# h2oai/datatable

Hardware: NVIDIA H100
Metric: rows/sec groupby-sum 1e9 int32 keys (higher is better)
Workload: dtype int32 keys / float64 sums

## Files before the change

### datatable_b200/csrc/dtb_api.cu

```cuda
#include <stdio.h>
#include <chrono>
#include <string.h>
#include <mutex>
#include <optional>
#include <string>
#include <vector>
#include "dtb_common.cuh"

namespace dtb {

static thread_local std::string t_error;
static thread_local dtb_call_stats t_stats = {0, 0, 0, 0, 0};

void set_error(const std::string& msg) { t_error = msg; }
void count_launch(int n) { t_stats.kernels_launched += n; }

static int64_t opt_radix_bits = 0;
static int64_t opt_verbose = 0;
static int64_t opt_profile = 0;
static int64_t opt_bucketed = 1;

struct ProfRec { const char* name; cudaEvent_t a, b; };
static thread_local std::vector<ProfRec> t_prof_open;
static thread_local std::vector<std::pair<std::string, double>> t_prof_done;
// ... 86 lines not shown
    if (slabs.size() > 1) {
      size_t total = 0;
      for (auto& sl : slabs) total += sl.cap;
      DTB_CUDA_CHECK(cudaDeviceSynchronize());
      for (auto& sl : slabs) cudaFree(sl.p);
      slabs.clear();
      char* p = nullptr;
      cudaError_t e = cudaMalloc(&p, total);
      if (e != cudaSuccess) { cudaGetLastError(); }
      else slabs.push_back({p, total});
    }
    cur = 0; off = 0;
    return DTB_OK;
  }
  void end() { if (depth > 0) depth--; }
  int take(size_t bytes, void** out) {
    bytes = (bytes + 255) & ~(size_t)255;
    while (cur < slabs.size()) {
      if (off + bytes <= slabs[cur].cap) { *out = slabs[cur].p + off; off += bytes; return DTB_OK; }
      cur++; off = 0;
    }
    size_t cap = bytes < ((size_t)64 << 20) ? ((size_t)64 << 20) : bytes;
    char* p = nullptr;
    cudaError_t e = cudaMalloc(&p, cap);
    if (e != cudaSuccess) {
      set_error("cudaMalloc(" + std::to_string(cap) + " bytes): " + cudaGetErrorString(e));
      cudaGetLastError();
      return e == cudaErrorMemoryAllocation ? DTB_ENOMEM : DTB_ECUDA;
    }
    slabs.push_back({p, cap});
// ... 258 lines not shown
  int     flags[MAX_KEYS];
  KeyPlan kp;
  int64_t nskip = 0;
  bool    groups_k = false;
  std::vector<RoundPlan> rounds;
  bool    fused_raw = false;
  int     buf_key_bytes = 4;
  int     dbits = 99;
  bool    direct_ok = false;
  bool    count_table = false;
  bool    fused_direct = false;
  int64_t ctable = 0;
  int64_t ftable = 0;
  std::vector<BucketCol> bcols;
  std::vector<int> bcol_of;
};

struct GroupBufs {
  DevIn  in[MAX_KEYS];
  const void* dptrs[MAX_KEYS];
  bool   staged = false;
  bool   fr_streamable = false;
  ColStats st[MAX_KEYS];
  DevBuf rawhist, rawna;
  DevBuf keyA, keyB, idxA, idxB, idxR0, idxR1;
  DevBuf gcount;
  DevBuf facc;
  DevBuf bxk;
  void*  sorted_keys = nullptr;
};

static int stage_inputs(const dtb_col* keys, int nkeys, int64_t n, const FusedReducers* fr, cudaStream_t s,
                        GroupBufs& b)
{
  for (int c = 0; c < nkeys; c++) {
    DTB_TRY(b.in[c].bind(keys[c].data, (size_t)n * stype_bytes(keys[c].stype), s));
    b.dptrs[c] = b.in[c].dptr;
    b.staged = b.staged || b.in[c].buf.p != nullptr;
  }
  b.fr_streamable = fr && fr->n > 0;
  for (int i = 0; b.fr_streamable && i < fr->n; i++)
    b.fr_streamable = fr->spec[i].op <= DTB_OP_NROWS &&
                       (fr->spec[i].op == DTB_OP_NROWS || is_device_ptr(fr->spec[i].value.data));
// ... 95 lines not shown
    const int np = r.pp.npasses;
    const int low = gp.count_table && np > 1 ? r.pp.shift[np - 1] : 0;
    const bool narrow = !r.want_sorted_keys && !(gp.count_table && (np > 3 || low > 16));
    r.low_bits = narrow ? low : 0;
    for (int p = 0; p < np; p++) {
      const bool lastp = p == np - 1;
      const int left = r.kp.total_bits - r.pp.shift[p] - r.pp.bits[p];
      r.kdrop[p] = narrow && p > 0 ? r.pp.shift[p] : 0;
      r.kin_bytes[p] = p == 0 ? r.key_bytes : r.kout_bytes[p - 1];
      r.kout_bytes[p] = lastp ? (r.want_sorted_keys ? r.key_bytes : 0)
                      : !narrow ? r.key_bytes : left <= 8 ? 1 : left <= 16 ? 2 : left <= 32 ? 4 : 8;
    }
    r.fold = nkeys == 1 && ri == 0 && gp.fused_raw && r.kp.k[0].cshift == 0 && r.kp.k[0].lshift == 0;
    r.keep_composite = !gp.bcols.empty() && !gp.fused_raw && nrounds == 1 && r.key_bytes == 4;
  }
}

static void print_plan(const GroupPlan& gp, int64_t n, int nkeys, const ColStats* st) {
  if (!opt_verbose) return;
  const int nrounds = (int)gp.rounds.size();
  fprintf(stderr, "[dtb200] group: n=%lld keys=%d bits=%d rounds=%d\n", (long long)n, nkeys, gp.kp.total_bits, nrounds);
  for (int c = 0; c < nkeys; c++)
    fprintf(stderr, "[dtb200]   key %d: stype=%d desc=%d bits=%d cshift=%d lshift=%d na=%llu\n", c,
            gp.kp.k[c].stype, gp.kp.k[c].desc, gp.kp.k[c].bits, gp.kp.k[c].cshift, gp.kp.k[c].lshift,
            (unsigned long long)st[c].nacount);
  for (int ri = 0; ri < nrounds; ri++) {
    const RoundPlan& r = gp.rounds[ri];
    std::string kw;
    for (int p = 0; p < r.pp.npasses; p++)
      kw += (p ? "," : "") + std::to_string(r.kin_bytes[p]) + ":" + std::to_string(r.kout_bytes[p]);
    fprintf(stderr, "[dtb200]   round %d: keys=%d bits=%d group_shift=%d passes=%d narrow_after=%d fold=%d count_table=%d"
            " key_bytes=%s low_bits=%d\n",
            ri, r.kp.nkeys, r.kp.total_bits, r.kp.group_shift, r.pp.npasses, r.narrow_after, (int)r.fold,
            (int)(gp.count_table && ri == nrounds - 1), kw.c_str(), r.low_bits);
  }
}

static int sort_rounds(const GroupPlan& gp, int64_t n, int nfused, int32_t* order, cudaStream_t s, GroupBufs& b)
{
  const int nrounds = (int)gp.rounds.size();
  DTB_TRY(b.keyA.alloc((size_t)n * gp.buf_key_bytes, s));
  DTB_TRY(b.keyB.alloc((size_t)n * gp.buf_key_bytes, s));
  DTB_TRY(b.idxA.alloc((size_t)n * 4, s));
  DTB_TRY(b.idxB.alloc((size_t)n * 4, s));
  if (nrounds > 1) { DTB_TRY(b.idxR0.alloc((size_t)n * 4, s)); }
  if (nrounds > 2) { DTB_TRY(b.idxR1.alloc((size_t)n * 4, s)); }
  if (gp.count_table) {
    DTB_TRY(b.gcount.alloc(sizeof(u32) * (size_t)gp.ctable, s));
    DTB_CUDA_CHECK(cudaMemsetAsync(b.gcount.p, 0, sizeof(u32) * (size_t)gp.ctable, s));
  }
  if (gp.fused_direct) DTB_TRY(b.facc.alloc(sizeof(u64) * (size_t)gp.ftable * 2 * (size_t)nfused, s));
  DTB_TL("scratch allocated");
  const int32_t* idx_cur = nullptr;
  for (int ri = 0; ri < nrounds; ri++) {
    const RoundPlan& r = gp.rounds[ri];
    const KeyPlan& rk = r.kp;
    const PassPlan& pp = r.pp;
    t_stats.radix_passes += pp.npasses;
    int src_kind = 1;
    if (r.keep_composite) DTB_TRY(b.bxk.alloc(sizeof(u32) * (size_t)n, s));
    if (!gp.fused_raw) {
      ProfScope ps("compose_keys", s);
      DTB_TRY(launch_compose_keys(rk, n, idx_cur, r.keep_composite ? b.bxk.p : b.keyA.p, r.key_bytes, s)); src_kind = 0;
    }

    DevBuf work; DTB_TRY(work.alloc(radix_pass_work_bytes(n), s));
// ... 16 lines not shown
      io.keys_in = kin;
      io.out_shift = last ? 0 : r.kdrop[p + 1] - r.kdrop[p];
      io.out_bytes = r.kout_bytes[p];
      if (r.fold && p == 0 && pp.shift[0] == 0) {
        io.raw_hist = b.rawhist.as<unsigned short>(); io.raw_na = b.rawna.as<unsigned short>();
      }
      if (r.low_bits) {
        if (p == 0) io.bases_out = pp.npasses == 2 ? low_base : regions;
        if (p == 1 && !last) { io.regions = regions; io.region_bits = pp.bits[0]; io.low_hist = low_base; }
        if (last) { io.low_base = low_base; io.low_bits = r.low_bits; }
      }
      io.idx_in = iin;
      io.keys_out = (last && !r.want_sorted_keys) ? nullptr : kout;
      int32_t* iout = last ? round_out : ((p & 1) ? b.idxB.as<int32_t>() : b.idxA.as<int32_t>());
      io.idx_out = iout;
      DTB_TRY(launch_radix_pass(io, rk, r.kin_bytes[p], n, pp.shift[p] - r.kdrop[p], pp.bits[p], work.as<u32>(), s,
                                (gp.count_table && last) ? b.gcount.as<u32>() : nullptr, rk.group_shift));
      if (last && r.want_sorted_keys) b.sorted_keys = kout;
      kin = kout;
      kout = (kout == b.keyA.p) ? b.keyB.p : b.keyA.p;
      iin = iout;
    }
    idx_cur = round_out;
  }
  return DTB_OK;
}

static int group_offsets(const GroupPlan& gp, int64_t n, const int32_t* order, int32_t* offsets, GroupBufs& b,
                         GroupResult& res, cudaStream_t s)
{
  if (res.ngroups < 0) return DTB_OK;
  if (!gp.groups_k) {
// ... 94 lines not shown
    const void* vals[BK_MAXCOLS]; int sts[BK_MAXCOLS]; unsigned long long* words[BK_MAXCOLS][BK_NWORDS];
    const int nc = sw.second - sw.first;
    for (int c = 0; c < nc; c++) {
      const BucketCol& bc = gp.bcols[sw.first + c];
      vals[c] = bc.data; sts[c] = bc.stype;
      for (int w = 0; w < BK_NWORDS; w++) words[c][w] = tables[(size_t)(sw.first + c) * BK_NWORDS + w];
    }
    DTB_TRY(launch_bucketed_reduce(b.bxk.as<u32>(), bshift, gp.dbits, nc, vals, sts, n, slab_starts,
                                   start, words, bscr.p, s));
  }
  return DTB_OK;
}

static int direct_reduce(const DirectGroups& dg, const DirectPlan& dp, int op, dtb_col value, const int32_t* order,
                         const int32_t* offsets, int64_t n, int64_t ng, u64* acc0, u64* acc1, bool accumulate,
                         void* out, cudaStream_t s)
{
  GroupRows rows;
  rows.v = value.data; rows.nv = n; rows.order = order; rows.offsets = offsets; rows.n = n;
  DevBuf zscr;
  if (minmax_zero_sign(op, value.stype)) { DTB_TRY(zscr.alloc(zero_fix_bytes(ng), s)); rows.zpos = zscr.as<u64>(); }
  if (accumulate && ng > 0) {
    ProfScope ps("reduce_direct", s);
    DTB_TRY(launch_direct_init(op, dp, dg.table, acc0, acc1, s));
    DTB_TRY(launch_direct_accumulate_rows(op, dg.kp, dp, value.data, value.stype, n, acc0, acc1, s));
  }
  return launch_direct_finalize(op, value.stype, acc0, acc1, dp, (const uint32_t*)dg.gkeys, ng, out, rows, s);
}

static int reduce_rowindex(int op, const void* value, int stype, int64_t nrows_value, const void* order, int order_is64,
                           const int32_t* offsets, int64_t ng, int64_t n, u64* acc, void* out, cudaStream_t s)
{
  DevBuf extra;
  const size_t xb = reduce_extra_bytes(op, stype, ng, n);
  if (xb) DTB_TRY(extra.alloc(xb, s));
  ProfScope ps("reduce", s);
  return launch_reduce_impl(op, value, stype, nrows_value, order, order_is64, offsets, ng, n, acc, acc + ng, out, s,
                            xb ? extra.p : nullptr);
}

// ... 15 lines not shown
  if (bucketed) DTB_TRY(bucketed_reduce(gp, n, b, tables, s));
  for (int i = 0; i < fr.n; i++) {
    const dtb_reduce_spec& sp = fr.spec[i];
    int out_st = 0;
    DTB_TRY(reducer_out_stype(sp.op, sp.value.stype, out_st));
    DevBuf ob; DTB_TRY(ob.alloc_owned((size_t)(ng > 0 ? ng : 1) * stype_bytes(out_st), s));
    if (sp.op == DTB_OP_NROWS) {
      DTB_TRY(launch_nrows(offsets, ng, ob.p, s));
    } else if (bucketed && gp.bcol_of[i] >= 0) {
      u64* const* w = &tables[(size_t)gp.bcol_of[i] * BK_NWORDS];
      const BucketWords bw = bucket_words(sp.op, sp.value.stype);
      DTB_TRY(direct_reduce(res.direct, dp, sp.op, sp.value, order, offsets, n, ng, w[bw.a0],
                            bw.a1 >= 0 ? w[bw.a1] : nullptr, false, ob.p, s));
    } else if (gp.fused_direct) {
      u64* acc = b.facc.as<u64>() + (size_t)gp.ftable * 2 * i;
      DTB_TRY(direct_reduce(res.direct, dp, sp.op, sp.value, order, offsets, n, ng, acc, acc + gp.ftable, true, ob.p, s));
    } else {
      DevIn dv;
      if (sp.op != DTB_OP_NROWS) DTB_TRY(dv.bind(sp.value.data, (size_t)n * stype_bytes(sp.value.stype), s));
      DTB_TRY(reduce_rowindex(sp.op, dv.dptr, sp.value.stype, n, order, 0, offsets, ng, n, gacc.as<u64>(), ob.p, s));
    }
    fr.out[i] = ob.detach();
  }
  return DTB_OK;
}

static int validate_group(const dtb_col* keys, int nkeys, const int* flags, int na_pos, int64_t n, bool handle,
                          bool wide)
{
  if (nkeys < 1 || nkeys > MAX_KEYS) { set_error("number of key columns must be in 1.." + std::to_string(MAX_KEYS)); return DTB_EINVAL; }
  if (!keys || !flags) { set_error("keys/flags must not be NULL"); return DTB_EINVAL; }
// ... 977 lines not shown
```

### datatable_b200/csrc/dtb_common.cuh

```cuda
#pragma once
#include <cuda_runtime.h>
#include <stdint.h>
#include <string.h>
#include <type_traits>
#include "dtb_internal.h"

namespace dtb {

constexpr int NUM_SMS = 132;

constexpr int PASS_THREADS = 256;
constexpr int PASS_IPT = 16;
constexpr int PASS_TILE = PASS_THREADS * PASS_IPT;
constexpr int CHUNK_TILES = 16;
constexpr int CHUNK_ROWS = PASS_TILE * CHUNK_TILES;

typedef unsigned long long u64;
typedef unsigned int u32;

template <typename T> struct NaOf;
template <> struct NaOf<int8_t>  { static __host__ __device__ int8_t  v() { return INT8_MIN;  } };
template <> struct NaOf<int16_t> { static __host__ __device__ int16_t v() { return INT16_MIN; } };
template <> struct NaOf<int32_t> { static __host__ __device__ int32_t v() { return INT32_MIN; } };
template <> struct NaOf<int64_t> { static __host__ __device__ int64_t v() { return INT64_MIN; } };
// ... 120 lines not shown
    } else {
      u64 u; const bool valid = RawKey<T>::get(r, u);
      return (KeyT)norm_apply(valid, u, k);
    }
  }
  __device__ __forceinline__ KeyT load(int64_t i) const { return norm(load_raw(i)); }
};

__device__ __forceinline__ u64 ld_relaxed_u64(const u64* p) {
  u64 v; asm volatile("ld.relaxed.gpu.global.u64 %0, [%1];" : "=l"(v) : "l"(p) : "memory"); return v;
}
__device__ __forceinline__ void st_relaxed_u64(u64* p, u64 v) {
  asm volatile("st.relaxed.gpu.global.u64 [%0], %1;" :: "l"(p), "l"(v) : "memory");
}

__device__ __forceinline__ unsigned lanemask_lt() {
  unsigned m; asm("mov.u32 %0, %%lanemask_lt;" : "=r"(m)); return m;
}

static inline int stype_bytes(int st) {
  switch (st) {
    case DTB_STYPE_BOOL: case DTB_STYPE_INT8: return 1;
    case DTB_STYPE_INT16: return 2;
    case DTB_STYPE_INT32: case DTB_STYPE_FLOAT32: case DTB_STYPE_DATE32: return 4;
    case DTB_STYPE_INT64: case DTB_STYPE_FLOAT64: case DTB_STYPE_TIME64: return 8;
    default: return 0;
  }
}

static inline int grid_for(int64_t blocks, int per_sm) {
// ... 27 lines not shown
```

### datatable_b200/csrc/dtb_internal.h

```cpp
#pragma once
#include <cuda_runtime.h>
#include <stdint.h>
#include <string>
#include "../../include/dtb200.h"

namespace dtb {

constexpr int MAX_KEYS = 8;
constexpr int MAX_PASSES = 16;

void set_error(const std::string& msg);
void count_launch(int n = 1);
struct ProfScope {
  ProfScope(const char* name, cudaStream_t s);
  ~ProfScope();
  bool on; cudaStream_t s; const char* name; cudaEvent_t a, b;
};

#define DTB_CUDA_CHECK(expr)                                                     \
  do {                                                                           \
    cudaError_t _e = (expr);                                                     \
    if (_e != cudaSuccess) {                                                     \
      ::dtb::set_error(std::string(#expr) + ": " + cudaGetErrorString(_e));      \
      return DTB_ECUDA;                                                          \
// ... 52 lines not shown
  int         src_kind;
  const void* keys_in;
  const int32_t* idx_in;
  void*       keys_out;
  int32_t*    idx_out;
  const unsigned short* raw_hist = nullptr;
  const unsigned short* raw_na = nullptr;
  int         out_shift = 0;
  int         out_bytes = 0;
  uint32_t*       bases_out = nullptr;
  const uint32_t* regions = nullptr;
  int             region_bits = 0;
  uint32_t*       low_hist = nullptr;
  const uint32_t* low_base = nullptr;
  int             low_bits = 0;
};

size_t radix_pass_work_bytes(int64_t n);
int launch_radix_pass(const PassIO& io, const KeyPlan& kp, int key_bytes, int64_t n,
                      int shift, int bits, uint32_t* work, cudaStream_t s,
                      uint32_t* group_count = nullptr, int group_shift = 0);

int launch_offsets_from_counts(const uint32_t* count, int64_t table, int64_t n, int32_t* offsets,
                               uint32_t* gkeys, unsigned long long* d_ngroups, unsigned long long* scratch,
                               cudaStream_t s);

int launch_dense_scatter(const void* keys, int key_bytes, const void* vals, int64_t n, int64_t kmin, int64_t size,
                         void* table, uint32_t* present, cudaStream_t s);
int launch_dense_emit(const uint32_t* gidx, const void* table, int64_t ng, int64_t kmin, int key_bytes,
                      void* out_keys, void* out_vals, cudaStream_t s);
// ... 18 lines not shown
size_t zero_fix_bytes(int64_t ngroups);
bool minmax_zero_sign(int op, int stype);

int launch_first_valid_pos(const void* v, int stype, int64_t nv, const void* order, int order_is64, const int32_t* offsets,
                           int64_t ngroups, int64_t n, int zero_only, const unsigned long long* gate,
                           unsigned long long* pos, cudaStream_t s);

int launch_reduce_impl(int op, const void* value, int stype, int64_t nrows_value,
                       const void* order, int order_is64, const int32_t* offsets, int64_t ngroups,
                       int64_t n, unsigned long long* acc0, unsigned long long* acc1,
                       void* out, cudaStream_t s, void* extra = nullptr);
size_t reduce_extra_bytes(int op, int stype, int64_t ng, int64_t n);
int reduce_out_stype_host(int op, int stype);
int launch_offsets_check(const int32_t* offsets, int64_t ng, int* d_bad, cudaStream_t s);

enum { DIRECT_PLAIN = 0,
       DIRECT_SMALL = 1,
       DIRECT_HOT = 2 };
struct DirectPlan {
  int kind;
  const void* map;
  int64_t nslots;
};
size_t direct_map_bytes(int64_t table);
int plan_direct(int64_t table, const uint32_t* gkeys, const int32_t* offsets, int64_t ngroups, int64_t n,
                int64_t gmax, void* map_scratch, cudaStream_t s, DirectPlan& dp);
int launch_direct_init(int op, const DirectPlan& dp, int64_t table, unsigned long long* acc0, unsigned long long* acc1, cudaStream_t s);
int launch_direct_accumulate_rows(int op, const KeyPlan& kp, const DirectPlan& dp, const void* value, int stype, int64_t n,
                                  unsigned long long* acc0, unsigned long long* acc1, cudaStream_t s);
int launch_direct_finalize(int op, int stype, const unsigned long long* acc0, const unsigned long long* acc1,
                           const DirectPlan& dp, const uint32_t* gkeys, int64_t ngroups, void* out, const GroupRows& rows,
                           cudaStream_t s);
int launch_inverse_order(const int32_t* order, int64_t n, int32_t* inv, cudaStream_t s);
int launch_first_zero_rows(const void* value_rows, int stype, int64_t row0, int64_t nrows, const int32_t* inv,
                           const int32_t* offsets, int64_t ngroups, unsigned long long* first_zero, cudaStream_t s);
int launch_nrows(const int32_t* offsets, int64_t ngroups, void* out, cudaStream_t s);
int launch_group_keys(const void* sorted_keys, int key_bytes, const int32_t* offsets, int group_shift,
                      int64_t ngroups, uint32_t* gkeys, cudaStream_t s);

enum { BK_SUMI = 0, BK_SUMF = 1, BK_CNT = 2, BK_MIN = 3, BK_MAX = 4, BK_CNTNA = 5, BK_NWORDS = 6 };
constexpr int BK_MAX_DBITS = 20, BK_MIN_DBITS = 12;
size_t bucket_starts_bytes(int64_t n);
int launch_bucket_starts(const uint32_t* xkeys, int gshift, int64_t n, int nb, uint32_t* slab_starts, uint32_t* bstart, cudaStream_t s);
constexpr int BK_MAXCOLS = 4;
// ... 56 lines not shown
```

### datatable_b200/csrc/dtb_radix.cu

```cuda
#include "dtb_common.cuh"

namespace dtb {

template <typename T>
__device__ __forceinline__ void compose_col4(const KeyNorm& k, const int64_t (&row)[4], const bool (&in)[4], u64 (&x)[4]) {
  typedef typename RawKey<T>::load_t L;
  L raw[4];
#pragma unroll
  for (int r = 0; r < 4; r++) raw[r] = in[r] ? ((const L*)k.data)[row[r]] : (L)0;
#pragma unroll
  for (int r = 0; r < 4; r++) {
    u64 u; const bool valid = RawKey<T>::get(raw[r], u);
    x[r] |= norm_apply(valid, u, k) << k.lshift;
  }
}

template <typename KeyT>
__global__ void __launch_bounds__(256)
compose_keys_kernel(KeyPlan kp, int64_t n, const int32_t* __restrict__ idx, KeyT* __restrict__ out, int out_shift)
{
  const int64_t stride = (int64_t)gridDim.x * blockDim.x * 4;
  for (int64_t i0 = (int64_t)blockIdx.x * blockDim.x * 4 + threadIdx.x; i0 < n; i0 += stride) {
    int64_t row[4]; bool in[4]; u64 x[4];
#pragma unroll
// ... 25 lines not shown
  if (key_bytes == 4 && kp.total_bits - out_shift > 32) {
    set_error("internal: a " + std::to_string(kp.total_bits - out_shift) + "-bit key does not fit 32 bits");
    return DTB_EINVAL;
  }
  if (n == 0) return DTB_OK;
  const int grid = grid_for((n + 1023) / 1024, 16);
  if (key_bytes == 4) compose_keys_kernel<u32><<<grid, 256, 0, s>>>(kp, n, idx, (u32*)keys_out, out_shift);
  else                compose_keys_kernel<u64><<<grid, 256, 0, s>>>(kp, n, idx, (u64*)keys_out, out_shift);
  count_launch();
  DTB_CUDA_CHECK(cudaGetLastError());
  return DTB_OK;
}


int64_t radix_num_chunks(int64_t n) { return (n + CHUNK_ROWS - 1) / CHUNK_ROWS; }

__device__ __forceinline__ u32 slot_owner(const u32* b, u32 lo, u32 hi, u32 s) {
  while (lo < hi) { const u32 mid = (lo + hi + 1) >> 1; if (b[mid] <= s) lo = mid; else hi = mid - 1; }
  return lo;
}

template <typename KeyT, typename Src, int NBINS>
__global__ void __launch_bounds__(PASS_THREADS)
count_kernel(const __grid_constant__ Src src, int64_t n, int shift, u32 mask, u32* __restrict__ counts,
             unsigned short* __restrict__ tile_pre, const u32* __restrict__ regions, int region_bits,
             u32* __restrict__ low_hist)
{
  constexpr int BPT = NBINS / PASS_THREADS;
  __shared__ u32 h[NBINS];
  __shared__ u32 rg[256];
  const int64_t cbase = (int64_t)blockIdx.x * CHUNK_ROWS;
  const int64_t cend = (cbase + CHUNK_ROWS < n) ? cbase + CHUNK_ROWS : n;
  const u32 rmax = (1u << region_bits) - 1;
  if (regions) { if (threadIdx.x <= rmax) rg[threadIdx.x] = regions[threadIdx.x]; }
  u32 total[BPT];
// ... 160 lines not shown
  KeyT*          keys_out;
  int32_t*       idx_out;
  int64_t        n;
  int            shift;
  u32            mask;
  const u32*     chunk_offs;
  const u32*     digit_base;
  const unsigned short* tile_pre;
  u32*           group_count;
  int            group_shift;
  int            out_shift;
  int            out_bytes;
  const u32*     low_base;
  int            low_bits;
  const uint2*   tile_low;
};

__device__ __forceinline__ void mbar_init(uint64_t* bar, u32 count) {
  const u32 a = (u32)__cvta_generic_to_shared(bar);
  asm volatile("mbarrier.init.shared::cta.b64 [%0], %1;" :: "r"(a), "r"(count) : "memory");
  asm volatile("fence.mbarrier_init.release.cluster;" ::: "memory");
}
__device__ __forceinline__ void tma_load_1d(void* smem_dst, const void* gsrc, u32 bytes, uint64_t* bar) {
  const u32 d = (u32)__cvta_generic_to_shared(smem_dst), b = (u32)__cvta_generic_to_shared(bar);
  asm volatile("mbarrier.arrive.expect_tx.shared::cta.b64 _, [%0], %1;" :: "r"(b), "r"(bytes) : "memory");
  asm volatile("cp.async.bulk.shared::cluster.global.mbarrier::complete_tx::bytes [%0], [%1], %2, [%3];"
               :: "r"(d), "l"(gsrc), "r"(bytes), "r"(b) : "memory");
}
__device__ __forceinline__ void mbar_wait(uint64_t* bar, u32 parity) {
  const u32 b = (u32)__cvta_generic_to_shared(bar);
// ... 160 lines not shown
      } else {
        skey[lp] = key[i];
        sidx[lp] = r;
      }
    }
  }
  __syncthreads();
}

template <typename KeyT>
__device__ __forceinline__ KeyT staged_key(const KeyT* skey, int q) {
  if constexpr (sizeof(KeyT) == 4) return (KeyT)reinterpret_cast<const uint2*>(skey)[q].x;
  else return skey[q];
}

template <typename KeyT, typename Src, int NBINS, int MINB, int NB>
__global__ void __launch_bounds__(PASS_THREADS, MINB)
scatter_kernel(const __grid_constant__ PassArgs<KeyT, Src> a)
{
  constexpr int THREADS = PASS_THREADS, TILE = PassCfg<KeyT, NBINS>::TILE, TILES = PassCfg<KeyT, NBINS>::TILES;
  constexpr int WARPS = THREADS / 32;
  constexpr int BPT = NBINS / THREADS;
  extern __shared__ __align__(16) unsigned char smem_raw[];
  __shared__ u32 s_wsum[WARPS];
  __shared__ __align__(8) uint64_t s_bar;
  u32* bin_dst    = reinterpret_cast<u32*>(smem_raw + sizeof(unsigned short) * WARPS * NBINS);
  KeyT* skey      = reinterpret_cast<KeyT*>(bin_dst + NBINS + 4);
  int32_t* sidx   = reinterpret_cast<int32_t*>(skey + TILE);

  const int tid = threadIdx.x;
  const int64_t base = (int64_t)blockIdx.x * TILE;
  const int tile_n = (int)((a.n - base) < (int64_t)TILE ? (a.n - base) : (int64_t)TILE);
  const int64_t tile = (int64_t)blockIdx.x * TILES;
  const int64_t chunk = tile / CHUNK_TILES;

  u32 bin_run[BPT];
#pragma unroll
  for (int j = 0; j < BPT; j++) {
    const int b = tid * BPT + j;
    bin_run[j] = a.digit_base[b] + a.chunk_offs[(size_t)chunk * NBINS + b] + (u32)a.tile_pre[(size_t)tile * NBINS + b];
  }
  uint2 tl = make_uint2(0, 0);
  if constexpr (Src::packed && sizeof(typename Src::raw_t) == 1) {
    if (a.low_base) {
      const int64_t last = tile + (tile_n - 1) / PASS_TILE;
      tl = make_uint2(a.tile_low[tile].x, a.tile_low[last].y);
    }
  }

  if (tile_n == TILE) scatter_tile<KeyT, Src, NBINS, true,  NB>(a, smem_raw, s_wsum, &s_bar, base, tile_n, bin_run, tl);
  else                scatter_tile<KeyT, Src, NBINS, false, NB>(a, smem_raw, s_wsum, &s_bar, base, tile_n, bin_run, tl);

  const int lane = tid & 31;
#pragma unroll 4
  for (int p0 = 0; p0 < tile_n; p0 += THREADS) {
    const int p = p0 + tid;
    const bool valid = p < tile_n;
    KeyT k = 0; int32_t rid = 0;
    if (valid) {
      if constexpr (sizeof(KeyT) == 4) {
        const uint2 kv = reinterpret_cast<const uint2*>(skey)[p];
        k = (KeyT)kv.x; rid = (int32_t)kv.y;
      } else {
        k = skey[p]; rid = sidx[p];
      }
    }
// ... 9 lines not shown
      }
    }
    if (valid) {
      const u32 d = (u32)(k >> a.shift) & a.mask;
      const u32 dst = bin_dst[d] + (u32)p;
      if (a.keys_out) {
        const KeyT ko = k >> a.out_shift;
        switch (a.out_bytes) {
          case 1:  reinterpret_cast<unsigned char*>(a.keys_out)[dst] = (unsigned char)ko; break;
          case 2:  reinterpret_cast<unsigned short*>(a.keys_out)[dst] = (unsigned short)ko; break;
          case 4:  reinterpret_cast<u32*>(a.keys_out)[dst] = (u32)ko; break;
          default: a.keys_out[dst] = ko; break;
        }
      }
      a.idx_out[dst] = rid;
    }
  }
}

template <typename KeyT, typename Src, int NBINS>
static int run_scatter(Src src, const PassIO& io, int64_t n, int shift, u32 mask, int64_t ntiles,
                       const u32* counts, const u32* base, const unsigned short* tile_counts,
                       u32* group_count, int group_shift, const uint2* tile_low, cudaStream_t s)
{
  constexpr int MINB = PassCfg<KeyT, NBINS>::MINB;
  PassArgs<KeyT, Src> a;
  a.src = src; a.idx_in = io.idx_in; a.keys_out = (KeyT*)io.keys_out; a.idx_out = io.idx_out;
  a.n = n; a.shift = shift + io.low_bits; a.mask = mask; a.chunk_offs = counts; a.digit_base = base;
  a.tile_pre = tile_counts; a.group_count = group_count; a.group_shift = group_shift;
  a.out_shift = io.out_shift; a.out_bytes = io.out_bytes ? io.out_bytes : (int)sizeof(KeyT);
  a.low_base = io.low_base; a.low_bits = io.low_bits; a.tile_low = tile_low;
  constexpr size_t smem = PassCfg<KeyT, NBINS>::SMEM;
  constexpr int TILE = PassCfg<KeyT, NBINS>::TILE;
  const int bits = __builtin_popcount(mask);
  void (*kern)(const PassArgs<KeyT, Src>) =
      bits <= 6 ? scatter_kernel<KeyT, Src, NBINS, MINB, 6>
    : bits == 7 ? scatter_kernel<KeyT, Src, NBINS, MINB, 7> : scatter_kernel<KeyT, Src, NBINS, MINB, 8>;
  DTB_CUDA_CHECK(cudaFuncSetAttribute(kern, cudaFuncAttributeMaxDynamicSharedMemorySize, (int)smem));
  ProfScope ps("radix_scatter", s);
  kern<<<(unsigned)((n + TILE - 1) / TILE), PASS_THREADS, smem, s>>>(a);
  count_launch();
  DTB_CUDA_CHECK(cudaGetLastError());
  return DTB_OK;
}

template <typename KeyT, typename Src, int NBINS>
static int run_pass_nb(Src src, const PassIO& io, int64_t n, int shift, int bits, u32* work, cudaStream_t s,
                       u32* group_count, int group_shift)
{
  const int64_t nchunks = radix_num_chunks(n);
  const int64_t ntiles = (n + PASS_TILE - 1) / PASS_TILE;
  u32* counts = work;
// ... 59 lines not shown
  const size_t nbins = 256;
  return sizeof(u32) * ((size_t)radix_num_chunks(n) * nbins + 2 * nbins)
       + sizeof(unsigned short) * (ntiles + CHUNK_TILES) * nbins + sizeof(uint2) * ntiles;
}

int launch_radix_pass(const PassIO& io, const KeyPlan& kp, int key_bytes, int64_t n,
                      int shift, int bits, uint32_t* work, cudaStream_t s,
                      uint32_t* group_count, int group_shift)
{
  if (bits < 1 || bits > 8) { set_error("internal: digit width must be 1..8 bits"); return DTB_EINVAL; }
  if ((io.low_base && (io.src_kind != 0 || key_bytes != 1 || io.low_bits < 1 || io.low_bits > 16)) ||
      (io.regions && (io.raw_hist || !io.low_hist || io.region_bits < 1 || io.region_bits + bits > 16)) ||
      io.out_bytes > (key_bytes == 8 ? 8 : 4)) {
    set_error("internal: bad key widths for a radix pass"); return DTB_EINVAL;
  }
  if (io.src_kind == 0) {
    switch (key_bytes) {
      case 1: { PackedSrc<unsigned char, u32> src{(const unsigned char*)io.keys_in};
        return run_pass<u32>(src, io, n, shift, bits, work, s, group_count, group_shift); }
      case 2: { PackedSrc<unsigned short, u32> src{(const unsigned short*)io.keys_in};
        return run_pass<u32>(src, io, n, shift, bits, work, s, group_count, group_shift); }
      case 4: { PackedSrc<u32> src{(const u32*)io.keys_in};
        return run_pass<u32>(src, io, n, shift, bits, work, s, group_count, group_shift); }
      default: { PackedSrc<u64> src{(const u64*)io.keys_in};
        return run_pass<u64>(src, io, n, shift, bits, work, s, group_count, group_shift); }
    }
  }
  return key_bytes == 4 ? run_pass_raw<u32>(io, kp, n, shift, bits, work, s, group_count, group_shift)
                        : run_pass_raw<u64>(io, kp, n, shift, bits, work, s, group_count, group_shift);
}
// ... 31 lines not shown
```

### datatable_b200/csrc/dtb_reduce.cu

```cuda
#include <type_traits>
#include "dtb_common.cuh"

namespace dtb {

enum { CAT_SUMI = 0, CAT_SUMF = 1, CAT_MEAN = 2, CAT_MINMAX = 3, CAT_COUNT = 4, CAT_PRODI = 5, CAT_PRODF = 6 };

constexpr int RT = 256;
constexpr int RIPT = 8;
constexpr int RTILE = RT * RIPT;

template <int CAT> struct Partial;
template <> struct Partial<CAT_SUMI> { u64 s; };
template <> struct Partial<CAT_SUMF> { double s; };
template <> struct Partial<CAT_MEAN> { double s; u32 c; };
template <> struct Partial<CAT_MINMAX> { u64 key; };
template <> struct Partial<CAT_COUNT> { u32 c; };
template <> struct Partial<CAT_PRODI> { u64 p; };
template <> struct Partial<CAT_PRODF> { double m; int64_t e; u32 f; };

constexpr u64 PRODF_FRAC = (1ull << 52) - 1;
__device__ __forceinline__ double prodf_sig(u64 w) {
  return __longlong_as_double((long long)((w & PRODF_FRAC) | 0x3FF0000000000000ull));
}
__device__ __forceinline__ void prodf_mul(Partial<CAT_PRODF>& a, double m, int64_t e, u32 f) {
// ... 1045 lines not shown
  if constexpr (CAT == CAT_SUMI) { if (a0) atomicAdd(&acc0[g], a0); }
  else if constexpr (CAT == CAT_SUMF) {
    const double d = __longlong_as_double((long long)a0);
    if (d != 0.0) atomicAdd(reinterpret_cast<double*>(acc0) + g, d);
  }
  else if constexpr (CAT == CAT_MEAN) {
    if (a1) { atomicAdd(reinterpret_cast<double*>(acc0) + g, __longlong_as_double((long long)a0)); atomicAdd(&acc1[g], a1); }
  }
  else if constexpr (CAT == CAT_MINMAX) {
    if (flag) { if (a0 != ~0ull) atomicMin(&acc0[g], a0); }
    else      { if (a0 != 0ull)  atomicMax(&acc0[g], a0); }
  }
  else { if (a0) atomicAdd(&acc0[g], a0); }
}

constexpr int SMALL_TABLE = 2048;

template <typename T, int CAT, typename KSrc>
__global__ void __launch_bounds__(512)
direct_reduce_small_kernel(KSrc ksrc, int gshift, const typename RawKey<T>::load_t* __restrict__ v,
                           int64_t n, int table, const uint16_t* __restrict__ dense,
                           u64* acc0, u64* acc1, int flag)
{
  __shared__ u64 s0[SMALL_TABLE];
  __shared__ u64 s1[SMALL_TABLE];
  const u64 ident = (CAT == CAT_MINMAX && flag) ? ~0ull : 0ull;
  const int copies = (table * 16 <= SMALL_TABLE) ? 16 : 1;
  const int wofs = (copies > 1) ? (int)(threadIdx.x >> 5) * table : 0;
  for (int i = threadIdx.x; i < table * copies; i += blockDim.x) { s0[i] = ident; s1[i] = 0; }
  __syncthreads();
  const int64_t stride = (int64_t)gridDim.x * blockDim.x;
// ... 176 lines not shown
  const int out_st = reduce_out_stype(op, stype);
  if (!out_st) { set_error("Invalid column type in reducer"); return DTB_EINVAL; }
  if (n <= 0) return DTB_OK;
  auto accumulate = [&](const auto& ks) {
    return with_stype(stype, "internal: reducer of stype ", [&](auto t) {
      return direct_op<typename decltype(t)::type>(dp, op, ks, kp.group_shift, value, n, acc0, acc1, s);
    });
  };
  if (kp.nkeys != 1) { DirectComposite ks; ks.kp = kp; return accumulate(ks); }
  return with_stype(kp.k[0].stype, "internal: key of stype ", [&](auto t) {
    DirectRawKey<typename decltype(t)::type> ks; ks.src.init(kp.k[0]);
    return accumulate(ks);
  });
}

int launch_direct_finalize(int op, int stype, const u64* acc0, const u64* acc1, const DirectPlan& dp,
                           const uint32_t* gkeys, int64_t ng, void* out, const GroupRows& rows, cudaStream_t s)
{
  return finalize(op, stype, acc0, acc1, (dp.kind == DIRECT_SMALL && dp.map) ? nullptr : gkeys, ng, out, rows, s);
}

__global__ void inverse_order_kernel(const int32_t* __restrict__ order, int64_t n, int32_t* __restrict__ inv) {
  const int64_t stride = (int64_t)gridDim.x * blockDim.x;
  for (int64_t p = (int64_t)blockIdx.x * blockDim.x + threadIdx.x; p < n; p += stride) inv[order[p]] = (int32_t)p;
}

int launch_inverse_order(const int32_t* order, int64_t n, int32_t* inv, cudaStream_t s) {
  if (n == 0) return DTB_OK;
  const int grid = grid_for((n + 255) / 256, 8);
  inverse_order_kernel<<<grid, 256, 0, s>>>(order, n, inv);
// ... 92 lines not shown
```

Before: 29.96 billion.

## Carry sum values through first radix pass and reduce per region in shared memory

The first radix scatter pass over a raw 32-bit key column now also permutes the sum value column into digit order, and records per-digit bases. A new region-sum kernel then walks each radix region sequentially and accumulates into a shared-memory table indexed by the narrowed low key bits, combining runs of equal keys with warp shuffles before flushing to global accumulators. This replaces random global atomics over the full direct table with mostly shared-memory atomics. The cost is an extra n-sized value buffer, extra writes in the scatter pass and more shared memory per scatter block, and it only applies to one SUM reducer under specific layout conditions.

```diff
diff --git a/datatable_b200/csrc/dtb_api.cu b/datatable_b200/csrc/dtb_api.cu
--- a/datatable_b200/csrc/dtb_api.cu
+++ b/datatable_b200/csrc/dtb_api.cu
@@ -124,6 +124,7 @@
     return DTB_OK;
   }
   void end() { if (depth > 0) depth--; }
+  size_t room() const { return cur < slabs.size() ? slabs[cur].cap - off : 0; }
   int take(size_t bytes, void** out) {
     bytes = (bytes + 255) & ~(size_t)255;
     while (cur < slabs.size()) {
@@ -412,6 +413,9 @@
   int64_t ftable = 0;
   std::vector<BucketCol> bcols;
   std::vector<int> bcol_of;
+  bool    region_sum = false;
+  int     region_col = -1;
+  dtb_col region_value = {};
 };
 
 struct GroupBufs {
@@ -425,6 +429,8 @@
   DevBuf gcount;
   DevBuf facc;
   DevBuf bxk;
+  DevBuf vperm, rbases;
+  void*  region_keys = nullptr;
   void*  sorted_keys = nullptr;
 };
 
@@ -550,6 +556,23 @@
     r.fold = nkeys == 1 && ri == 0 && gp.fused_raw && r.kp.k[0].cshift == 0 && r.kp.k[0].lshift == 0;
     r.keep_composite = !gp.bcols.empty() && !gp.fused_raw && nrounds == 1 && r.key_bytes == 4;
   }
+
+  if (gp.fused_direct && gp.fused_raw && gp.bcols.empty() && gp.ftable > SMALL_TABLE) {
+    const RoundPlan& r = gp.rounds[0];
+    const int np = r.pp.npasses;
+    const bool layout = np >= 2 && np <= 3 && r.pp.shift[0] == 0 && r.kp.group_shift == 0 && r.kdrop[1] == r.pp.bits[0] &&
+                        (r.kout_bytes[0] == 1 || r.kout_bytes[0] == 2) && gp.dbits - r.pp.bits[0] <= REGION_MAX_LBITS;
+    for (int i = 0; layout && i < fr->n; i++)
+      if (fr->spec[i].op == DTB_OP_SUM && reduce_out_stype_host(DTB_OP_SUM, fr->spec[i].value.stype)) {
+        gp.region_sum = true; gp.region_col = i; gp.region_value = fr->spec[i].value;
+        break;
+      }
+  }
+}
+
+static bool takes_region_sum(const GroupPlan& gp, const dtb_reduce_spec& sp) {
+  return gp.region_sum && sp.op == DTB_OP_SUM && sp.value.data == gp.region_value.data &&
+         sp.value.stype == gp.region_value.stype;
 }
 
 static void print_plan(const GroupPlan& gp, int64_t n, int nkeys, const ColStats* st) {
@@ -570,9 +593,12 @@
             ri, r.kp.nkeys, r.kp.total_bits, r.kp.group_shift, r.pp.npasses, r.narrow_after, (int)r.fold,
             (int)(gp.count_table && ri == nrounds - 1), kw.c_str(), r.low_bits);
   }
-}
-
-static int sort_rounds(const GroupPlan& gp, int64_t n, int nfused, int32_t* order, cudaStream_t s, GroupBufs& b)
+  if (gp.region_sum)
+    fprintf(stderr, "[dtb200]   region_sum: reducer=%d stype=%d regions=%d bits_per_region=%d\n", gp.region_col,
+            gp.region_value.stype, 1 << gp.rounds[0].pp.bits[0], gp.dbits - gp.rounds[0].pp.bits[0]);
+}
+
+static int sort_rounds(GroupPlan& gp, int64_t n, int nfused, int32_t* order, cudaStream_t s, GroupBufs& b)
 {
   const int nrounds = (int)gp.rounds.size();
   DTB_TRY(b.keyA.alloc((size_t)n * gp.buf_key_bytes, s));
@@ -586,6 +612,22 @@
     DTB_CUDA_CHECK(cudaMemsetAsync(b.gcount.p, 0, sizeof(u32) * (size_t)gp.ctable, s));
   }
   if (gp.fused_direct) DTB_TRY(b.facc.alloc(sizeof(u64) * (size_t)gp.ftable * 2 * (size_t)nfused, s));
+  if (gp.region_sum) {
+    const size_t arena_cur = t_arena.cur, arena_off = t_arena.off;
+    const int64_t scratch0 = t_stats.scratch_bytes;
+    const size_t later = sizeof(u64) * 8 * (size_t)gp.ftable + ((size_t)64 << 20);
+    size_t free_b = 0, total_b = 0;
+    bool ok = b.rbases.alloc(sizeof(u32) * 256, s) == DTB_OK &&
+              b.vperm.alloc((size_t)n * stype_bytes(gp.region_value.stype), s) == DTB_OK;
+    if (ok && t_arena.room() < later) ok = cudaMemGetInfo(&free_b, &total_b) == cudaSuccess && free_b >= later;
+    if (!ok) {
+      cudaGetLastError();
+      gp.region_sum = false;
+      t_arena.cur = arena_cur; t_arena.off = arena_off;
+      t_stats.scratch_bytes = scratch0;
+      set_error("");
+    }
+  }
   DTB_TL("scratch allocated");
   const int32_t* idx_cur = nullptr;
   for (int ri = 0; ri < nrounds; ri++) {
@@ -632,8 +674,16 @@
       io.keys_out = (last && !r.want_sorted_keys) ? nullptr : kout;
       int32_t* iout = last ? round_out : ((p & 1) ? b.idxB.as<int32_t>() : b.idxA.as<int32_t>());
       io.idx_out = iout;
+      const bool carry = gp.region_sum && p == 0;
+      if (carry) {
+        io.vals = gp.region_value.data; io.vperm = b.vperm.p; io.vbytes = stype_bytes(gp.region_value.stype);
+        if (!io.bases_out) io.bases_out = b.rbases.as<u32>();
+        b.region_keys = kout;
+      }
       DTB_TRY(launch_radix_pass(io, rk, r.kin_bytes[p], n, pp.shift[p] - r.kdrop[p], pp.bits[p], work.as<u32>(), s,
                                 (gp.count_table && last) ? b.gcount.as<u32>() : nullptr, rk.group_shift));
+      if (carry && io.bases_out != b.rbases.p)
+        DTB_CUDA_CHECK(cudaMemcpyAsync(b.rbases.p, io.bases_out, sizeof(u32) * 256, cudaMemcpyDeviceToDevice, s));
       if (last && r.want_sorted_keys) b.sorted_keys = kout;
       kin = kout;
       kout = (kout == b.keyA.p) ? b.keyB.p : b.keyA.p;
@@ -758,7 +808,7 @@
 
 static int direct_reduce(const DirectGroups& dg, const DirectPlan& dp, int op, dtb_col value, const int32_t* order,
                          const int32_t* offsets, int64_t n, int64_t ng, u64* acc0, u64* acc1, bool accumulate,
-                         void* out, cudaStream_t s)
+                         void* out, cudaStream_t s, const GroupPlan* region = nullptr, const GroupBufs* rb = nullptr)
 {
   GroupRows rows;
   rows.v = value.data; rows.nv = n; rows.order = order; rows.offsets = offsets; rows.n = n;
@@ -767,7 +817,16 @@
   if (accumulate && ng > 0) {
     ProfScope ps("reduce_direct", s);
     DTB_TRY(launch_direct_init(op, dp, dg.table, acc0, acc1, s));
-    DTB_TRY(launch_direct_accumulate_rows(op, dg.kp, dp, value.data, value.stype, n, acc0, acc1, s));
+    if (region) {
+      const bool hot = dp.kind == DIRECT_HOT;
+      ProfScope pr(hot ? "region_sum_hot" : "region_sum", s);
+      const RoundPlan& r = region->rounds[0];
+      DTB_TRY(launch_region_sum(rb->region_keys, r.kout_bytes[0], r.pp.bits[0], region->dbits - r.pp.bits[0],
+                                (const u32*)rb->rbases.p, rb->vperm.p, value.stype, n,
+                                hot ? (const uint8_t*)dp.map : nullptr, acc0, s));
+    } else {
+      DTB_TRY(launch_direct_accumulate_rows(op, dg.kp, dp, value.data, value.stype, n, acc0, acc1, s));
+    }
   }
   return launch_direct_finalize(op, value.stype, acc0, acc1, dp, (const uint32_t*)dg.gkeys, ng, out, rows, s);
 }
@@ -813,7 +872,11 @@
                             bw.a1 >= 0 ? w[bw.a1] : nullptr, false, ob.p, s));
     } else if (gp.fused_direct) {
       u64* acc = b.facc.as<u64>() + (size_t)gp.ftable * 2 * i;
-      DTB_TRY(direct_reduce(res.direct, dp, sp.op, sp.value, order, offsets, n, ng, acc, acc + gp.ftable, true, ob.p, s));
+      const bool region = takes_region_sum(gp, sp) && dp.kind != DIRECT_SMALL;
+      if (opt_verbose && takes_region_sum(gp, sp))
+        fprintf(stderr, "[dtb200]   reducer %d: %s\n", i, region ? "region sum" : "direct (few groups)");
+      DTB_TRY(direct_reduce(res.direct, dp, sp.op, sp.value, order, offsets, n, ng, acc, acc + gp.ftable, true, ob.p, s,
+                            region ? &gp : nullptr, &b));
     } else {
       DevIn dv;
       if (sp.op != DTB_OP_NROWS) DTB_TRY(dv.bind(sp.value.data, (size_t)n * stype_bytes(sp.value.stype), s));
diff --git a/datatable_b200/csrc/dtb_common.cuh b/datatable_b200/csrc/dtb_common.cuh
--- a/datatable_b200/csrc/dtb_common.cuh
+++ b/datatable_b200/csrc/dtb_common.cuh
@@ -158,6 +158,11 @@
   asm volatile("st.relaxed.gpu.global.u64 [%0], %1;" :: "l"(p), "l"(v) : "memory");
 }
 
+__device__ __forceinline__ u32 slot_owner(const u32* b, u32 lo, u32 hi, u32 s) {
+  while (lo < hi) { const u32 mid = (lo + hi + 1) >> 1; if (b[mid] <= s) lo = mid; else hi = mid - 1; }
+  return lo;
+}
+
 __device__ __forceinline__ unsigned lanemask_lt() {
   unsigned m; asm("mov.u32 %0, %%lanemask_lt;" : "=r"(m)); return m;
 }
diff --git a/datatable_b200/csrc/dtb_internal.h b/datatable_b200/csrc/dtb_internal.h
--- a/datatable_b200/csrc/dtb_internal.h
+++ b/datatable_b200/csrc/dtb_internal.h
@@ -90,6 +90,9 @@
   uint32_t*       low_hist = nullptr;
   const uint32_t* low_base = nullptr;
   int             low_bits = 0;
+  const void*     vals = nullptr;
+  void*           vperm = nullptr;
+  int             vbytes = 0;
 };
 
 size_t radix_pass_work_bytes(int64_t n);
@@ -138,6 +141,7 @@
 int reduce_out_stype_host(int op, int stype);
 int launch_offsets_check(const int32_t* offsets, int64_t ng, int* d_bad, cudaStream_t s);
 
+constexpr int SMALL_TABLE = 2048;
 enum { DIRECT_PLAIN = 0,
        DIRECT_SMALL = 1,
        DIRECT_HOT = 2 };
@@ -152,6 +156,9 @@
 int launch_direct_init(int op, const DirectPlan& dp, int64_t table, unsigned long long* acc0, unsigned long long* acc1, cudaStream_t s);
 int launch_direct_accumulate_rows(int op, const KeyPlan& kp, const DirectPlan& dp, const void* value, int stype, int64_t n,
                                   unsigned long long* acc0, unsigned long long* acc1, cudaStream_t s);
+constexpr int REGION_MAX_LBITS = 13;
+int launch_region_sum(const void* lkey, int key_bytes, int rbits, int lbits, const uint32_t* bases, const void* vperm,
+                      int stype, int64_t n, const uint8_t* hot, unsigned long long* acc0, cudaStream_t s);
 int launch_direct_finalize(int op, int stype, const unsigned long long* acc0, const unsigned long long* acc1,
                            const DirectPlan& dp, const uint32_t* gkeys, int64_t ngroups, void* out, const GroupRows& rows,
                            cudaStream_t s);
diff --git a/datatable_b200/csrc/dtb_radix.cu b/datatable_b200/csrc/dtb_radix.cu
--- a/datatable_b200/csrc/dtb_radix.cu
+++ b/datatable_b200/csrc/dtb_radix.cu
@@ -63,11 +63,6 @@
 
 
 int64_t radix_num_chunks(int64_t n) { return (n + CHUNK_ROWS - 1) / CHUNK_ROWS; }
-
-__device__ __forceinline__ u32 slot_owner(const u32* b, u32 lo, u32 hi, u32 s) {
-  while (lo < hi) { const u32 mid = (lo + hi + 1) >> 1; if (b[mid] <= s) lo = mid; else hi = mid - 1; }
-  return lo;
-}
 
 template <typename KeyT, typename Src, int NBINS>
 __global__ void __launch_bounds__(PASS_THREADS)
@@ -258,6 +253,9 @@
   const u32*     low_base;
   int            low_bits;
   const uint2*   tile_low;
+  const void*    vals;
+  void*          vperm;
+  int            vbytes;
 };
 
 __device__ __forceinline__ void mbar_init(uint64_t* bar, u32 count) {
@@ -448,19 +446,47 @@
   else return skey[q];
 }
 
-template <typename KeyT, typename Src, int NBINS, int MINB, int NB>
+template <typename W>
+__device__ __forceinline__ void carry_values(const W* __restrict__ vals, W* __restrict__ vperm, int64_t base, int tile_n,
+                                             const unsigned short* inv, const unsigned char* dig, const u32* bin_dst,
+                                             W* sv)
+{
+  constexpr int VB = 16;
+  for (int p0 = 0; p0 < tile_n; p0 += PASS_THREADS * VB) {
+    W w[VB];
+#pragma unroll
+    for (int j = 0; j < VB; j++) {
+      const int pos = p0 + j * PASS_THREADS + (int)threadIdx.x;
+      w[j] = pos < tile_n ? vals[base + pos] : (W)0;
+    }
+#pragma unroll
+    for (int j = 0; j < VB; j++) {
+      const int pos = p0 + j * PASS_THREADS + (int)threadIdx.x;
+      if (pos < tile_n) sv[inv[pos]] = w[j];
+    }
+  }
+  __syncthreads();
+#pragma unroll 4
+  for (int p = threadIdx.x; p < tile_n; p += PASS_THREADS) vperm[bin_dst[dig[p]] + (u32)p] = sv[p];
+}
+
+template <typename KeyT, typename Src, int NBINS, int MINB, int NB, bool VALS>
 __global__ void __launch_bounds__(PASS_THREADS, MINB)
 scatter_kernel(const __grid_constant__ PassArgs<KeyT, Src> a)
 {
   constexpr int THREADS = PASS_THREADS, TILE = PassCfg<KeyT, NBINS>::TILE, TILES = PassCfg<KeyT, NBINS>::TILES;
   constexpr int WARPS = THREADS / 32;
   constexpr int BPT = NBINS / THREADS;
+  static_assert(!VALS || (sizeof(KeyT) == 4 && !Src::packed && PassCfg<KeyT, NBINS>::USE_RIDX),
+                "values travel in the first pass over a raw column with 32-bit keys, staged in the row-id buffer");
   extern __shared__ __align__(16) unsigned char smem_raw[];
   __shared__ u32 s_wsum[WARPS];
   __shared__ __align__(8) uint64_t s_bar;
   u32* bin_dst    = reinterpret_cast<u32*>(smem_raw + sizeof(unsigned short) * WARPS * NBINS);
   KeyT* skey      = reinterpret_cast<KeyT*>(bin_dst + NBINS + 4);
   int32_t* sidx   = reinterpret_cast<int32_t*>(skey + TILE);
+  unsigned short* inv = reinterpret_cast<unsigned short*>(sidx + TILE);
+  unsigned char* dig  = reinterpret_cast<unsigned char*>(inv + TILE);
 
   const int tid = threadIdx.x;
   const int64_t base = (int64_t)blockIdx.x * TILE;
@@ -484,6 +510,11 @@
 
   if (tile_n == TILE) scatter_tile<KeyT, Src, NBINS, true,  NB>(a, smem_raw, s_wsum, &s_bar, base, tile_n, bin_run, tl);
   else                scatter_tile<KeyT, Src, NBINS, false, NB>(a, smem_raw, s_wsum, &s_bar, base, tile_n, bin_run, tl);
+  if constexpr (VALS) {
+    const char* vp = reinterpret_cast<const char*>(a.vals) + base * a.vbytes;
+    for (int l = tid; l < (tile_n * a.vbytes + 127) / 128; l += THREADS)
+      asm volatile("prefetch.global.L2 [%0];" :: "l"(vp + (size_t)l * 128));
+  }
 
   const int lane = tid & 31;
 #pragma unroll 4
@@ -523,6 +554,16 @@
         }
       }
       a.idx_out[dst] = rid;
+      if constexpr (VALS) { inv[(u32)rid - (u32)base] = (unsigned short)p; dig[p] = (unsigned char)d; }
+    }
+  }
+  if constexpr (VALS) {
+    __syncthreads();
+    switch (a.vbytes) {
+      case 1:  carry_values((const uint8_t*)a.vals, (uint8_t*)a.vperm, base, tile_n, inv, dig, bin_dst, (uint8_t*)skey); break;
+      case 2:  carry_values((const uint16_t*)a.vals, (uint16_t*)a.vperm, base, tile_n, inv, dig, bin_dst, (uint16_t*)skey); break;
+      case 4:  carry_values((const u32*)a.vals, (u32*)a.vperm, base, tile_n, inv, dig, bin_dst, (u32*)skey); break;
+      default: carry_values((const u64*)a.vals, (u64*)a.vperm, base, tile_n, inv, dig, bin_dst, (u64*)skey); break;
     }
   }
 }
@@ -539,12 +580,21 @@
   a.tile_pre = tile_counts; a.group_count = group_count; a.group_shift = group_shift;
   a.out_shift = io.out_shift; a.out_bytes = io.out_bytes ? io.out_bytes : (int)sizeof(KeyT);
   a.low_base = io.low_base; a.low_bits = io.low_bits; a.tile_low = tile_low;
+  a.vals = io.vals; a.vperm = io.vperm; a.vbytes = io.vbytes;
   constexpr size_t smem = PassCfg<KeyT, NBINS>::SMEM;
   constexpr int TILE = PassCfg<KeyT, NBINS>::TILE;
   const int bits = __builtin_popcount(mask);
   void (*kern)(const PassArgs<KeyT, Src>) =
-      bits <= 6 ? scatter_kernel<KeyT, Src, NBINS, MINB, 6>
-    : bits == 7 ? scatter_kernel<KeyT, Src, NBINS, MINB, 7> : scatter_kernel<KeyT, Src, NBINS, MINB, 8>;
+      bits <= 6 ? scatter_kernel<KeyT, Src, NBINS, MINB, 6, false>
+    : bits == 7 ? scatter_kernel<KeyT, Src, NBINS, MINB, 7, false> : scatter_kernel<KeyT, Src, NBINS, MINB, 8, false>;
+  if (io.vals) {
+    if constexpr (sizeof(KeyT) == 4 && !Src::packed) {
+      kern = bits <= 6 ? scatter_kernel<KeyT, Src, NBINS, MINB, 6, true>
+           : bits == 7 ? scatter_kernel<KeyT, Src, NBINS, MINB, 7, true> : scatter_kernel<KeyT, Src, NBINS, MINB, 8, true>;
+    } else {
+      set_error("internal: values travel only in the first pass over a raw column with 32-bit keys"); return DTB_EINVAL;
+    }
+  }
   DTB_CUDA_CHECK(cudaFuncSetAttribute(kern, cudaFuncAttributeMaxDynamicSharedMemorySize, (int)smem));
   ProfScope ps("radix_scatter", s);
   kern<<<(unsigned)((n + TILE - 1) / TILE), PASS_THREADS, smem, s>>>(a);
@@ -634,6 +684,10 @@
       io.out_bytes > (key_bytes == 8 ? 8 : 4)) {
     set_error("internal: bad key widths for a radix pass"); return DTB_EINVAL;
   }
+  if (io.vals && (io.src_kind != 1 || io.idx_in || !io.vperm || (io.vbytes != 1 && io.vbytes != 2 && io.vbytes != 4 &&
+                                                                  io.vbytes != 8))) {
+    set_error("internal: bad value column for a radix pass"); return DTB_EINVAL;
+  }
   if (io.src_kind == 0) {
     switch (key_bytes) {
       case 1: { PackedSrc<unsigned char, u32> src{(const unsigned char*)io.keys_in};
diff --git a/datatable_b200/csrc/dtb_reduce.cu b/datatable_b200/csrc/dtb_reduce.cu
--- a/datatable_b200/csrc/dtb_reduce.cu
+++ b/datatable_b200/csrc/dtb_reduce.cu
@@ -1083,7 +1083,6 @@
   else { if (a0) atomicAdd(&acc0[g], a0); }
 }
 
-constexpr int SMALL_TABLE = 2048;
 
 template <typename T, int CAT, typename KSrc>
 __global__ void __launch_bounds__(512)
@@ -1290,6 +1289,121 @@
   });
 }
 
+constexpr int REGION_THREADS = 256;
+constexpr int REGION_IPT = 8;
+
+template <int CAT>
+__device__ __forceinline__ void warp_key_sums(const Partial<CAT>& part, u32 key, bool join, int lane, u64* tab) {
+  for (unsigned m = __ballot_sync(0xffffffffu, join); m; m = __ballot_sync(0xffffffffu, join)) {
+    const int src = __ffs(m) - 1;
+    const u32 kk = __shfl_sync(0xffffffffu, key, src);
+    const bool mine = join && key == kk;
+    Partial<CAT> t; p_init(t, 0);
+    if (mine) t = part;
+#pragma unroll
+    for (int o = 16; o > 0; o >>= 1) t.s += __shfl_xor_sync(0xffffffffu, t.s, o);
+    if (lane == src) p_flush(t, (int64_t)kk, tab, nullptr, 0);
+    join = join && !mine;
+  }
+}
+
+template <typename T, int CAT, typename KW, bool HOT>
+__global__ void __launch_bounds__(REGION_THREADS, 3)
+region_sum_kernel(const KW* __restrict__ lkey, const typename RawKey<T>::load_t* __restrict__ v,
+                  const u32* __restrict__ bases, int rbits, int lbits, int64_t n, int64_t per,
+                  const uint8_t* __restrict__ hot, u64* acc0)
+{
+  typedef typename RawKey<T>::load_t L;
+  extern __shared__ u64 tab[];
+  __shared__ u32 rb[256];
+  const int tid = threadIdx.x, lane = tid & 31;
+  const int nl = 1 << lbits;
+  rb[tid] = bases[tid];
+  const int64_t s_end = ((int64_t)blockIdx.x + 1) * per < n ? ((int64_t)blockIdx.x + 1) * per : n;
+  for (int i = tid; i < nl; i += REGION_THREADS) tab[i] = 0;
+  __syncthreads();
+  for (int64_t s0 = (int64_t)blockIdx.x * per; s0 < s_end;) {
+    const u32 d = slot_owner(rb, 0, 255, (u32)s0);
+    const int64_t rend = d < 255 ? (int64_t)rb[d + 1] : n;
+    const int64_t e = rend < s_end ? rend : s_end;
+    for (int64_t i0 = s0; i0 < e; i0 += REGION_THREADS * REGION_IPT) {
+      KW k[REGION_IPT]; L w[REGION_IPT];
+#pragma unroll
+      for (int j = 0; j < REGION_IPT; j++) {
+        const int64_t i = i0 + j * REGION_THREADS + tid;
+        k[j] = i < e ? lkey[i] : (KW)0;
+        w[j] = i < e ? v[i] : (L)0;
+      }
+      Partial<CAT> part[REGION_IPT];
+      u32 jm = 0;
+#pragma unroll
+      for (int j = 0; j < REGION_IPT; j++) {
+        const bool in = i0 + j * REGION_THREADS + tid < e;
+        p_init(part[j], 0);
+        p_add<T, CAT>(part[j], w[j], in, 0);
+        const u32 x = (u32)k[j], up = __shfl_up_sync(0xffffffffu, x, 1);
+        bool join = in && lane > 0 && up == x;
+        if constexpr (HOT) join = join || (in && hot[(x << rbits) | d]);
+        jm |= (u32)join << j;
+      }
+      if (__any_sync(0xffffffffu, jm != 0)) {
+#pragma unroll
+        for (int j = 0; j < REGION_IPT; j++)
+          if (__any_sync(0xffffffffu, (jm >> j) & 1u)) warp_key_sums(part[j], (u32)k[j], (jm >> j) & 1u, lane, tab);
+      }
+#pragma unroll
+      for (int j = 0; j < REGION_IPT; j++)
+        if (!((jm >> j) & 1u)) p_flush(part[j], (int64_t)k[j], tab, nullptr, 0);
+    }
+    __syncthreads();
+    for (int i = tid; i < nl; i += REGION_THREADS) {
+      slot_flush<CAT>(tab[i], 0, ((int64_t)i << rbits) | d, acc0, nullptr, 0);
+      tab[i] = 0;
+    }
+    __syncthreads();
+    s0 = e;
+  }
+}
+
+template <typename T, typename KW, bool HOT>
+static void run_region_sum(const void* lkey, int rbits, int lbits, const uint32_t* bases, const void* vperm, int64_t n,
+                           const uint8_t* hot, u64* acc0, cudaStream_t s, cudaError_t& err)
+{
+  constexpr int CAT = std::is_floating_point<T>::value ? CAT_SUMF : CAT_SUMI;
+  typedef typename RawKey<T>::load_t L;
+  auto kern = region_sum_kernel<T, CAT, KW, HOT>;
+  const int smem = (int)sizeof(u64) << lbits;
+  err = cudaFuncSetAttribute(kern, cudaFuncAttributeMaxDynamicSharedMemorySize, smem);
+  if (err != cudaSuccess) return;
+  const int grid = grid_for((n + 65535) / 65536, 3);
+  const int64_t per = (n + grid - 1) / grid;
+  kern<<<grid, REGION_THREADS, smem, s>>>((const KW*)lkey, (const L*)vperm, bases, rbits, lbits, n, per, hot, acc0);
+  err = cudaGetLastError();
+}
+
+int launch_region_sum(const void* lkey, int key_bytes, int rbits, int lbits, const uint32_t* bases, const void* vperm,
+                      int stype, int64_t n, const uint8_t* hot, u64* acc0, cudaStream_t s)
+{
+  if ((key_bytes != 1 && key_bytes != 2) || lbits < 1 || lbits > REGION_MAX_LBITS || lbits > 8 * key_bytes ||
+      rbits < 1 || rbits > 8 || rbits + lbits > 22) {
+    set_error("internal: bad region sum layout"); return DTB_EINVAL;
+  }
+  if (n <= 0) return DTB_OK;
+  cudaError_t err = cudaSuccess;
+  const int rc = with_stype(stype, "internal: region sum of stype ", [&](auto t) {
+    typedef typename decltype(t)::type T;
+    if (key_bytes == 1) { if (hot) run_region_sum<T, uint8_t, true>(lkey, rbits, lbits, bases, vperm, n, hot, acc0, s, err);
+                          else     run_region_sum<T, uint8_t, false>(lkey, rbits, lbits, bases, vperm, n, hot, acc0, s, err); }
+    else                { if (hot) run_region_sum<T, uint16_t, true>(lkey, rbits, lbits, bases, vperm, n, hot, acc0, s, err);
+                          else     run_region_sum<T, uint16_t, false>(lkey, rbits, lbits, bases, vperm, n, hot, acc0, s, err); }
+    return DTB_OK;
+  });
+  DTB_TRY(rc);
+  count_launch();
+  DTB_CUDA_CHECK(err);
+  return DTB_OK;
+}
+
 int launch_direct_finalize(int op, int stype, const u64* acc0, const u64* acc1, const DirectPlan& dp,
                            const uint32_t* gkeys, int64_t ng, void* out, const GroupRows& rows, cudaStream_t s)
 {
```

New measurement: 31.76 billion (median of 6 runs). +6.0%, better.
